# thomasfork/aircraft_trajectory_optimization

Hardware: AMD Instinct MI355X
Metric: SQP iters/sec (batched) + lap-time err vs CasADi, 50×4 collocation (higher is better)
Workload: dtype f64; 1 GPU; racetrack_parametric_esp_drone_colloc_N50_K4_cold_start_batched_sqp; N=50, K=4, nz=13, nu=4, batch_per_gpu=512, global_batch=512, max_iter=47, layout=interleaved, parallelism=instances sharded x1

## Files before the change

### aircraft_trajectory_optimization_amd/csrc/ato_ipm.hip

```cpp
#include <hip/hip_runtime.h>
#include <cmath>
#include <string>
#include "../../include/ato_ipm.h"
#include "../../include/ato.h"

void ato_internal_set_error(const std::string& msg);

namespace {

constexpr int CH = 32;
constexpr int CB = 64;
constexpr int QMAX = 9;

__device__ __forceinline__ double nmax(double a, double b) {
    return (a != a || b != b) ? __builtin_nan("") : (a > b ? a : b);
}
__device__ __forceinline__ double nmin(double a, double b) {
    return (a != a || b != b) ? __builtin_nan("") : (a < b ? a : b);
}
__device__ __forceinline__ bool fin(double v) { return fabs(v) < INFINITY; }

struct Parts {
    int len[4];
    int c0[5];
// ... 580 lines not shown
        filter_reset_step(o, t, n, c, last, k1);
        if (t.ok) {
            ka = k;
            arm = t.arm_case;
            break;
        }
        al = al * 0.5;
    }
    fr_n[p] = n;
    fr_cnt[p] = c;
    fr_last[p] = last ? 1 : 0;
    nf[p] = k1;
    kacc[p] = ka;
    fail_out[p] = fl ? 1 : 0;
    arm_out[p] = arm ? 1 : 0;
}

__global__ __launch_bounds__(256) void k_kkt_diag(Dev d, const double* __restrict__ Sx, const double* __restrict__ Ss,
                                                  const double* __restrict__ dw, const double* __restrict__ dc,
                                                  double* __restrict__ dx, double* __restrict__ dr,
                                                  double* __restrict__ Ds) {
    const long long t = (long long)blockIdx.x * 256 + threadIdx.x;
    const long long nW = (long long)d.n * d.W, iW = (long long)d.mi * d.W, eW = (long long)d.meq * d.W;
    if (t < nW) {
        const int b = (int)(t % d.W);
        dx[t] = Sx[t] + dw[b];
    } else if (t < nW + iW) {
        const long long u = t - nW;
        const int r = (int)(u / d.W), b = (int)(u - (long long)r * d.W);
        const double ds = Ss[u] + dw[b];
// ... 564 lines not shown
    const int k0 = blockIdx.y * RROWS, k1 = min(n0 + m, k0 + RROWS);
    for (int k = k0 + (threadIdx.x >> 6); k < k1; k += 4) {
        const long long o = (long long)k * W + b;
        if (k < n0) {
            x[o] = xb[o];
        } else {
            const long long d = (long long)(k - n0) * W + b;
            const double y = xb[o], rp = x[o], rn = x[o + (long long)m * W];
            x[o] = (rp + y) / dp[d];
            x[o + (long long)m * W] = (rn - y) / dn[d];
            x[o + 2LL * m * W] = y;
        }
    }
}

}

extern "C" {

int ato_ipm_perturb(int32_t op, int32_t W, int32_t m, const double* prm, int64_t* hdeg, int64_t* jdeg,
                    int64_t* diters, int64_t* test, double* dx, double* dc, double* dx_last, double* dc_last,
                    const double* mu, uint8_t* pend, const int32_t* inertia, double* dw_out, double* dc_out,
                    uint8_t* tosolve, const uint8_t* fin, void* stream) {
    if (op < 0 || op > 2 || W < 0 || !prm) return fail(ATO_ERR_ARG, "ato_ipm_perturb: arguments");
    if (W == 0) return 0;
    if (!hdeg || !jdeg || !diters || !test || !dx || !dc || !dx_last || !dc_last || !mu || !pend ||
        (op == 1 && (!inertia || !dw_out || !dc_out || !tosolve)) || (op == 2 && (!tosolve || !fin)))
        return fail(ATO_ERR_ARG, "ato_ipm_perturb: arguments");
    const PertPrm o{prm[0], prm[1], prm[2], prm[3], prm[4], prm[5], prm[6], prm[7], (long long)prm[8]};
    hipLaunchKernelGGL(k_perturb, dim3((W + CB - 1) / CB), dim3(CB), 0, static_cast<hipStream_t>(stream), (int)op, W,
                       m, o, reinterpret_cast<long long*>(hdeg), reinterpret_cast<long long*>(jdeg),
                       reinterpret_cast<long long*>(diters), reinterpret_cast<long long*>(test), dx, dc, dx_last,
                       dc_last, mu, pend, inertia, dw_out, dc_out, tosolve, fin);
// ... 321 lines not shown
```

### aircraft_trajectory_optimization_amd/native.py

```python
import ctypes
import os
from typing import Optional, Tuple

import numpy as np

KMAX = 9
GEOM_WIDTH = 16

ATO_MODEL_DRONE, ATO_MODEL_POINT = 0, 1
ATO_ATT_ESP, ATO_ATT_YPR, ATO_ATT_DCM = 0, 1, 2
ATO_FRAME_GLOBAL, ATO_FRAME_PARAMETRIC = 0, 1
ATO_TRANS_COLLOCATION, ATO_TRANS_RK4 = 0, 1
ATO_GATE_CIRCLE, ATO_GATE_SQUARE = 0, 1
ATO_LAYOUT_INTERLEAVED, ATO_LAYOUT_INSTANCE_MAJOR = 0, 1
ATO_OK, ATO_ERR_ARG, ATO_ERR_UNSUPPORTED, ATO_ERR_HIP, ATO_ERR_STATE = 0, -1, -2, -3, -4
ABI_VERSION = 3
CPC_MAX = 16

_c_double_p = ctypes.POINTER(ctypes.c_double)


class AtoGate(ctypes.Structure):
    _fields_ = [
        ('interval', ctypes.c_int32),
# ... 60 lines not shown

class AtoIpmDims(ctypes.Structure):
    _fields_ = [('n', ctypes.c_int32), ('m', ctypes.c_int32), ('mi', ctypes.c_int32), ('meq', ctypes.c_int32),
                ('iin', ctypes.c_void_p), ('ieq', ctypes.c_void_p), ('W', ctypes.c_int32)]


class AtoIpmBounds(ctypes.Structure):
    _fields_ = [('xL', ctypes.c_void_p), ('xU', ctypes.c_void_p), ('dL', ctypes.c_void_p), ('dU', ctypes.c_void_p)]


IPM_SYMBOLS = ('ato_ipm_work_size', 'ato_ipm_errors', 'ato_ipm_rhs', 'ato_ipm_direction', 'ato_ipm_measures',
               'ato_ipm_multipliers', 'ato_ipm_filter_accept', 'ato_ipm_kkt_diag', 'ato_ipm_perturb',
               'ato_ipm_status', 'ato_ipm_barrier', 'ato_ipm_filter_multi', 'ato_ipm_refine_work',
               'ato_ipm_refine_pass', 'ato_ipm_refine_decide', 'ato_ipm_resto_rows', 'ato_ipm_js_jty',
               'ato_ipm_kmul_residual', 'ato_ipm_resto_eval', 'ato_ipm_resto_hess', 'ato_ipm_resto_kkt_pack',
               'ato_ipm_resto_kkt_diag', 'ato_ipm_resto_kkt_rhs', 'ato_ipm_resto_kkt_expand')

EXPORTED_SYMBOLS = ('ato_create', 'ato_destroy', 'ato_sizes', 'ato_sparsity', 'ato_bounds',
                    'ato_reserve', 'ato_eval', 'ato_eval_f32', 'ato_hess_sparsity', 'ato_hess_eval',
                    'ato_mesh_create', 'ato_mesh_destroy', 'ato_mesh_signed_distance',
                    'ato_timing', 'ato_timing_read', 'ato_timing_stride', 'ato_last_error', 'ato_version',
                    'ato_kkt_create', 'ato_kkt_destroy', 'ato_kkt_reserve', 'ato_kkt_factor', 'ato_kkt_solve',
                    'ato_kkt_residual', 'ato_kkt_residual_list', 'ato_set_instance_spheres',
                    'ato_sphere_rows', 'ato_gradf_mode', 'ato_gradf_sparsity', 'ato_replay_set_lift',
                    'ato_replay', 'ato_remesh') + IPM_SYMBOLS


def library_path() -> str:
    return os.environ.get('ATO_LIB_PATH') or os.path.join(os.path.dirname(os.path.abspath(__file__)), '_lib',
                                                          'libato.so')

# ... 53 lines not shown
        lib.ato_ipm_perturb.argtypes = [ctypes.c_int32] * 3 + [vp] * 16 + [vp]
        lib.ato_ipm_status.argtypes = [ctypes.c_int32] + [vp] * 11 + [vp]
        lib.ato_ipm_barrier.argtypes = [ctypes.c_int32] + [vp] * 10 + [vp]
        lib.ato_ipm_refine_work.argtypes = [ctypes.c_int32, ctypes.c_int32]
        lib.ato_ipm_refine_pass.argtypes = [ctypes.c_int32, ctypes.c_int32] + [vp] * 7 + [vp]
        lib.ato_ipm_refine_decide.argtypes = [ctypes.c_int32] * 4 + [vp] * 12 + [vp]
        lib.ato_ipm_resto_rows.argtypes = [ctypes.c_int32, ctypes.c_int32] + [vp] * 5 + [vp]
        lib.ato_ipm_js_jty.argtypes = [ctypes.c_int32] * 3 + [vp] * 8 + [vp]
        lib.ato_ipm_kmul_residual.argtypes = [ctypes.c_int32] * 5 + [vp] * 15 + [vp]
        lib.ato_ipm_resto_eval.argtypes = [ctypes.c_int32] * 5 + [vp] * 10 + [d] + [vp] * 3 + [vp]
        lib.ato_ipm_resto_hess.argtypes = [ctypes.c_int32] * 2 + [vp] * 7 + [vp]
        lib.ato_ipm_resto_kkt_pack.argtypes = [ctypes.c_int32] * 4 + [vp] * 9 + [vp]
        lib.ato_ipm_resto_kkt_diag.argtypes = [ctypes.c_int32] * 3 + [vp] * 9 + [vp]
        lib.ato_ipm_resto_kkt_rhs.argtypes = [ctypes.c_int32] * 3 + [vp] * 4 + [vp]
        lib.ato_ipm_resto_kkt_expand.argtypes = [ctypes.c_int32] * 3 + [vp] * 5 + [vp]
        for fn in IPM_SYMBOLS[1:]:
            getattr(lib, fn).restype = ctypes.c_int
        for fn in ('ato_create', 'ato_destroy', 'ato_sizes', 'ato_sparsity', 'ato_bounds', 'ato_reserve',
                   'ato_eval', 'ato_eval_f32', 'ato_hess_sparsity', 'ato_hess_eval', 'ato_timing',
                   'ato_timing_read', 'ato_timing_stride', 'ato_mesh_create', 'ato_mesh_destroy', 'ato_mesh_signed_distance',
                   'ato_set_instance_spheres', 'ato_sphere_rows', 'ato_gradf_mode', 'ato_gradf_sparsity',
                   'ato_replay_set_lift', 'ato_replay', 'ato_remesh'):
            getattr(lib, fn).restype = ctypes.c_int
    return lib


_LIB: Optional[ctypes.CDLL] = None


def load(path: Optional[str] = None) -> ctypes.CDLL:
# ... 225 lines not shown
```

### aircraft_trajectory_optimization_amd/solver/batched_ipm.py

```python
import os
import time
from dataclasses import dataclass, field
from typing import Dict, List, Optional

import numpy as np
import torch

from aircraft_trajectory_optimization_amd.solver.ipm import DEG_NO, DEG_UNKNOWN, DEG_YES, INF, IPMOptions, \
    T_C0X0, T_C0XP, T_CPX0, T_CPXP, T_NONE

RUNNING, OPTIMAL, ACCEPTABLE, MAX_ITER, LS_FAILED, KKT_FAILED, STOPPED, INACTIVE, TINY_STEP = range(9)
STATUS_NAMES = {RUNNING: 'running', OPTIMAL: 'optimal', ACCEPTABLE: 'acceptable', MAX_ITER: 'max_iter',
                LS_FAILED: 'restoration_failed', KKT_FAILED: 'kkt_failure', STOPPED: 'stopped',
                INACTIVE: 'inactive', TINY_STEP: 'tiny_step'}
WD_VECS = ('x', 's', 'y', 'zl', 'zu', 'vl', 'vu', 'dx', 'ds', 'dy', 'dzl', 'dzu', 'dvl', 'dvu')
WD_SCAL = ('alpha_max', 'alpha_z', 'theta', 'phi', 'gphi_d')
CSTAT = ('watchdog_started', 'watchdog_reverted', 'soft_resto_steps', 'resto_iterations', 'kkt_failures')
FILTER_MAX = 256


@dataclass
class BatchedIPMResult:
    x: torch.Tensor
    f: torch.Tensor
# ... 588 lines not shown
        al = alpha0.clone()
        for k in range(K):
            inval = act & ~(al > alpha_min)
            failed = failed | inval
            act = act & ~inval
            ok, armk = self._accept(theta, phi, gphi_d, al, tht[k], pht[k], F, nf, theta_min=theta_min, pend=act,
                                    frs=frs, theta_max=theta_max)
            kacc = torch.where(ok, torch.full_like(kacc, k), kacc)
            arm = torch.where(ok, armk, arm)
            act = act & ~ok
            al = al * 0.5
        return kacc, failed, arm

    LS_MULTI_K = int(os.environ.get('ATO_LS_MULTI_K', '8'))
    FUSED_RESTO = os.environ.get('ATO_IPM_FUSED_RESTO', '1') != '0'

    @staticmethod
    def _halvings(K, device):
        return torch.tensor([0.5 ** k for k in range(K)], dtype=torch.float64, device=device)

    def _multi_round(self, idx, P, K, x, s, dx, ds, alpha, alpha_min, mu, theta, phi, gphi_d, F, nf, frs):
        import copy
        cols = idx.repeat(K)
        pw = self._halvings(K + 1, alpha.device)[:K]
        ak = alpha.index_select(0, idx)[None, :] * pw[:, None]
        akf = ak.reshape(-1)
        Xm = x.index_select(1, cols) + akf * dx.index_select(1, cols)
        Sm = s.index_select(1, cols) + akf * ds.index_select(1, cols)
        view = copy.copy(self)
        if self.vk is not None:
            for k in ('sf', 'sg', 'c_rhs', 'xL', 'xU', 'dL', 'dU'):
                t = getattr(self, k)
                if torch.is_tensor(t) and t.dim() >= 1 and t.shape[-1] == self.B:
                    setattr(view, k, t.index_select(t.dim() - 1, cols).contiguous())
        else:
            view._compact(cols, ())
        view.B = K * P
        view.ev = getattr(self.ev, 'trial_subset', getattr(self.ev, 'subset', None))(K * P, cols)
        fm, gm = view._eval_fg(Xm)
        tht, pht = view._measures(Xm, Sm, gm, fm, mu.index_select(0, cols))
        sel = lambda t: t.index_select(0, idx)
        nf_p = sel(nf)
        frs_p = tuple(sel(t) for t in frs)
        kacc, failed, arm = self._filter_multi(sel(theta), sel(phi), sel(gphi_d), sel(alpha), sel(alpha_min),
                                               tht.reshape(K, P).contiguous(), pht.reshape(K, P).contiguous(),
                                               F.index_select(0, idx), nf_p, sel(self.theta_max), sel(self.theta_min),
                                               frs_p)
        nf.index_copy_(0, idx, nf_p)
        for t, tp in zip(frs, frs_p):
            t.index_copy_(0, idx, tp)
        lss = self.stats.setdefault('ls_multi', [0, 0])
        lss[0] += 1
        lss[1] += K * P
        return kacc, failed, arm

    def _filter_test(self, theta, phi, gphi_d, alpha, tht, pht, F, nf, pend, first, frs, theta_min=None):
        tmin = self.theta_min if theta_min is None else theta_min
        if self.vk is not None:
            return self.vk.filter_accept(theta, phi, gphi_d, alpha, tht, pht, F, nf, self.theta_max, tmin, pend,
                                         first, self.o, frs=frs)
        ok, arm = self._accept(theta, phi, gphi_d, alpha, tht, pht, F, nf, theta_min=tmin, pend=pend, frs=frs)
        return ok, arm, pend & ~ok & first & (tht >= theta)

    def _solve(self, rhs, mask, H, Js, dx, dr, idx=None):
        if idx is None:
            idx = _idx(mask)
        x = rhs.clone()
        if len(idx) == 0:
# ... 500 lines not shown
                        self._bd(), x, s, dx, ds, zl, zu, vl, vu, gx, gs, mu, tau)
                else:
                    dzl = torch.where(self.hxl, mu / a - zl - zl / a * dx, 0.0)
                    dzu = torch.where(self.hxu, mu / b - zu + zu / b * dx, 0.0)
                    dvl = torch.where(self.hsl, mu / c - vl - vl / c * ds, 0.0)
                    dvu = torch.where(self.hsu, mu / d - vu + vu / d * ds, 0.0)
                    alpha_max = torch.minimum(
                        torch.minimum(self._ftb(a, dx, self.hxl, tau), self._ftb(b, -dx, self.hxu, tau)),
                        torch.minimum(self._ftb(c, ds, self.hsl, tau), self._ftb(d, -ds, self.hsu, tau)))
                    alpha_z = torch.minimum(
                        torch.minimum(self._ftb(zl, dzl, self.hxl, tau), self._ftb(zu, dzu, self.hxu, tau)),
                        torch.minimum(self._ftb(vl, dvl, self.hsl, tau), self._ftb(vu, dvu, self.hsu, tau)))
                    gphi_d = (gx * dx).sum(0) + (gs * ds).sum(0)
                theta, phi = self._measures(x, s, g, f, mu)
                tiny = torch.zeros_like(act)
                if o.tiny_step_tol > 0:
                    rel_x = (dx.abs() / (1.0 + x.abs())).amax(0) if n else torch.zeros_like(mu)
                    rel_s = (ds.abs() / (1.0 + s.abs())).amax(0) if ds.shape[0] else torch.zeros_like(mu)
                    dymax = dy.abs().amax(0) if m else torch.zeros_like(mu)
                    tiny = act & ~in_wd & ~kwd & (rel_x <= o.tiny_step_tol) & (rel_s <= o.tiny_step_tol) & \
                        (dymax <= o.tiny_step_y_tol) & (theta <= 1e-4)
                    tiny_flag = tiny_flag | tiny
                soft_now = act & in_soft & ~tiny
                soft_count = torch.where(soft_now, soft_count + 1, soft_count)
                soft_over = soft_now & (soft_count > o.max_soft_resto_iters)
                soft_try = soft_now & ~soft_over
                dirs = {'dx': dx, 'ds': ds, 'dy': dy, 'dzl': dzl, 'dzu': dzu, 'dvl': dvl, 'dvu': dvu}
                nosoc = torch.zeros_like(act)
                wdm = torch.zeros_like(act)
                any_kwd = any_wd = False
                if wd_on:
                    start = act & ~tiny & ~in_wd & ~kwd & ~in_soft & (ws_short >= o.watchdog_shortened_iter_trigger)
                    wdm = act & ~kwd & (in_wd | start)
                    any_start, any_kwd, any_wd = torch.stack([start.any(), kwd.any(), wdm.any()]).tolist()
# ... 19 lines not shown
                                                                           ('vu', vu)))
                    for k in dirs:
                        dirs[k] = torch.where(m2, wd[k], dirs[k])
                    alpha_max, alpha_z, theta, phi, gphi_d = (
                        torch.where(msk, wd[k], v) for k, v in (('alpha_max', alpha_max), ('alpha_z', alpha_z),
                                                                ('theta', theta), ('phi', phi), ('gphi_d', gphi_d)))
                    in_wd = in_wd & ~msk
                    nosoc = nosoc | msk
                    fe_, ge_, gfe_, jve_ = self._eval(x)
                    f, g = torch.where(msk, fe_, f), torch.where(m2, ge_, g)
                    gf, jv = torch.where(m2, gfe_, gf), torch.where(m2, jve_, jv)
                    wdst[2] += msk.sum()
                    cst[1] += msk.long()

                def alpha_min_of(theta_, gphi_):
                    neg = gphi_ < 0
                    mgd = torch.clamp(-gphi_, min=1e-300)
                    t1 = o.gamma_phi * theta_ / mgd
                    t2 = o.delta * theta_ ** o.s_theta / mgd ** o.s_phi
                    amin = torch.where(neg & (theta_ <= self.theta_min),
                                       torch.clamp(torch.minimum(t1, t2), max=o.gamma_theta),
                                       torch.where(neg, torch.clamp(t1, max=o.gamma_theta),
                                                   torch.full_like(t1, o.gamma_theta)))
                    return o.alpha_min_frac * amin

                if any_kwd:
                    revert(kwd)
                dx, ds, dy, dzl, dzu, dvl, dvu = (dirs[k] for k in ('dx', 'ds', 'dy', 'dzl', 'dzu', 'dvl', 'dvu'))
                alpha_min = alpha_min_of(theta, gphi_d)
                alpha = torch.where(kwd, alpha_max * 0.5, alpha_max) if any_kwd else alpha_max.clone()
                wd_succ = torch.zeros_like(act)
                wd_cols = wdm.clone()
                pend = act & ~soft_now
                resto = torch.zeros(B, dtype=torch.bool, device=dev)
                first = torch.ones(B, dtype=torch.bool, device=dev)
                xn, sn = x.clone(), s.clone()
                an, dyn = torch.zeros_like(alpha), dy.clone()
                armn = torch.zeros(B, dtype=torch.bool, device=dev)
                fresh = pend.clone()
                fresh_any = True
                accf = torch.zeros(B, dtype=torch.bool, device=dev)
                frs = (fr_n, fr_cnt, fr_last)

                def take(mask, al, xt, st, arm, dyt):
                    nonlocal xn, sn, an, dyn, armn, accf
                    m2 = mask[None, :]
                    xn = torch.where(m2, xt, xn)
                    sn = torch.where(m2, st, sn)
                    an = torch.where(mask, al, an)
                    dyn = torch.where(m2, dyt, dyn)
                    armn = torch.where(mask, arm, armn)
                    accf = torch.where(mask, fresh, accf)

                laps.lap('direction')
                lsfail = torch.zeros_like(act)
                for _ls in range(200):
                    failed = pend & ~(alpha > alpha_min)
                    if o.ls_first_trial:
                        failed = failed & ~fresh
                    any_failed, n_left = torch.stack([failed.any(), (pend & ~failed).sum()]).tolist()
                    if any_failed:
                        lsfail = lsfail | failed
                        pend = pend & ~failed
                    if not n_left:
                        break
                    lss = self.stats.setdefault('ls_trials', [0, 0, 0])
                    lss[0] += 1
                    lss[1] += int(n_left)
                    lss[2] += int(_ls == 0)
                    K = self.LS_MULTI_K
                    if K > 0 and _ls >= 1 and not fresh_any and getattr(self.ev, 'trial_subset_ok',
                                                                          hasattr(self.ev, 'subset')):
                        pidx = torch.nonzero(pend).reshape(-1)
                        kacc, mfail, marm = self._multi_round(pidx, int(n_left), K, x, s, dx, ds, alpha, alpha_min,
                                                              mu, theta, phi, gphi_d, F, nf, frs)
                        acc_p = kacc >= 0
                        a_p = alpha.index_select(0, pidx) * self._halvings(K + 1, dev).index_select(
                            0, torch.where(acc_p, kacc, K).long())
                        acc = torch.zeros_like(pend).index_copy(0, pidx, acc_p)
                        mf = torch.zeros_like(pend).index_copy(0, pidx, mfail)
                        alpha = alpha.index_copy(0, pidx, a_p)
                        take(acc, alpha, x + alpha * dx, s + alpha * ds, torch.zeros_like(pend).index_copy(0, pidx, marm),
                             dy)
                        lsfail = lsfail | mf
                        pend = pend & ~acc & ~mf
                        continue
                    xt = x + alpha * dx
                    st = s + alpha * ds
                    laps.lap('ls_logic')
                    ft, gt = self._eval_fg(xt)
                    laps.lap('ls_eval')
                    tht, pht = self._measures(xt, st, gt, ft, mu)
                    if _ls == 0 and any_wd:
                        th_r, ph_r = torch.where(wdm, wd['theta'], theta), torch.where(wdm, wd['phi'], phi)
                        gd_r, al_r = torch.where(wdm, wd['gphi_d'], gphi_d), torch.where(wdm, wd['alpha_max'], alpha)
                    else:
                        th_r, ph_r, gd_r, al_r = theta, phi, gphi_d, alpha
                    okt, armt, soc = self._filter_test(th_r, ph_r, gd_r, al_r, tht, pht, F, nf,
                                                       pend & ~tiny if _ls == 0 else pend, first, frs)
                    soc = soc & ~nosoc & ~wdm & ~tiny
                    take(okt, alpha, xt, st, armt, dy)
                    pend = pend & ~okt
                    if _ls == 0:
# ... 718 lines not shown
```

### aircraft_trajectory_optimization_amd/solver/ipm_device.py

```python
import ctypes
from typing import Dict, Tuple

import numpy as np
import torch

from aircraft_trajectory_optimization_amd import native


def _p(t):
    return ctypes.c_void_p(t.data_ptr()) if t is not None else None


def resto_rows(dr, dp, dn):
    m, W = dr.shape
    for t in (dr, dp, dn):
        if t.dtype != torch.float64 or t.shape != (m, W) or not t.is_cuda:
            raise ValueError('resto_rows: expected fp64 [m, W] device tensors')
    dr, dp, dn = dr.contiguous(), dp.contiguous(), dn.contiguous()
    drow = torch.empty_like(dr)
    cnt = torch.zeros((W, 2), dtype=torch.int32, device=dr.device)
    lib = native.load()
    rc = lib.ato_ipm_resto_rows(m, W, _p(dr), _p(dp), _p(dn), _p(drow), _p(cnt),
                                ctypes.c_void_p(torch.cuda.current_stream(dr.device).cuda_stream))
    if rc != 0:
# ... 361 lines not shown
        self._own(frs[0], torch.int64, P, 'filter reset count')
        self._own(frs[1], torch.int64, P, 'filter reset trigger count')
        self._own(frs[2], torch.bool, P, 'filter rejection flag')
        key = ('filter', o.s_phi, o.s_theta, o.delta, o.eta_phi, o.gamma_theta, o.gamma_phi, o.obj_max_inc,
               o.compare_tol, o.max_filter_resets, o.filter_reset_trigger)
        prm = self._host_prm(key)
        kacc = torch.empty(P, dtype=torch.int32, device=self.device)
        out = torch.empty((2, P), dtype=torch.bool, device=self.device)
        th, ph, gd, a0, amin, tmax, tmin = cols
        self._check(self.lib.ato_ipm_filter_multi(P, K, F.shape[1], _p(th), _p(ph), _p(gd), _p(a0), _p(amin), _p(tht),
                                                  _p(pht), _p(F), _p(nf), _p(tmax), _p(tmin), prm.ctypes.data,
                                                  _p(frs[0]), _p(frs[1]), _p(frs[2]), _p(kacc), _p(out[0]),
                                                  _p(out[1]), self._stream()), 'ato_ipm_filter_multi')
        return kacc, out[0], out[1]

    def _refine_vec(self, t, N, W, what):
        if t.dtype != torch.float64 or t.device != self.device or t.shape != (N, W) or not t.is_contiguous():
            raise ValueError(f'refinement {what}: expected contiguous fp64 [{N}, {W}] on {self.device}')
        return t

    def refine_begin(self, rhs, x, res, mask, o):
        N, W = rhs.shape
        for t, w in ((rhs, 'rhs'), (x, 'x'), (res, 'residual')):
            self._refine_vec(t, N, W, w)
        self._own(mask, torch.bool, W, 'solved-column mask')
        nch = int(self.lib.ato_ipm_refine_work(N, W))
        f64 = dict(dtype=torch.float64, device=self.device)
        u8 = dict(dtype=torch.bool, device=self.device)
        key = ('refine', o.residual_ratio_max, o.residual_ratio_singular, o.min_refinement_steps,
               o.max_refinement_steps)
# ... 100 lines not shown
```

### include/ato_ipm.h

```cpp
#ifndef ATO_IPM_H
#define ATO_IPM_H

#include <stddef.h>
#include <stdint.h>

#ifdef __cplusplus
extern "C" {
#endif

typedef struct ato_ipm_dims {
    int32_t n;
    int32_t m;
    int32_t mi;
    int32_t meq;
    const int32_t* iin;
    const int32_t* ieq;
    int32_t W;
} ato_ipm_dims;

typedef struct ato_ipm_bounds {
    const double* xL;
    const double* xU;
    const double* dL;
    const double* dU;
// ... 76 lines not shown
                       const double* jv, const double* sg, const double* x_ref, const double* dr2,
                       const double* zeta, double rho, double* gr, double* gfr, double* jr, void* stream);
int ato_ipm_resto_hess(int32_t nnz, int32_t W, const int32_t* src, const int32_t* dcol, const double* H0,
                       const double* sigma, const double* zeta, const double* dr2, double* h, void* stream);
int ato_ipm_resto_kkt_pack(int32_t nh, int32_t nj, int32_t n0, int32_t W, const int32_t* h_map,
                           const int32_t* pos_orig, const int32_t* h_diag, const uint8_t* diag_new, const double* H,
                           const double* J, double* Hb, double* Jb, double* hd, void* stream);
int ato_ipm_resto_kkt_diag(int32_t n0, int32_t m, int32_t W, const double* dx, const double* dr, const double* hd,
                           const uint8_t* mask, double* dxb, double* drow, double* dp, double* dn, int32_t* cnt,
                           void* stream);
int ato_ipm_resto_kkt_rhs(int32_t n0, int32_t m, int32_t W, const double* x, const double* dp, const double* dn,
                          double* xb, void* stream);
int ato_ipm_resto_kkt_expand(int32_t n0, int32_t m, int32_t W, const double* xb, const double* dp, const double* dn,
                             const uint8_t* mask, double* x, void* stream);

#ifdef __cplusplus
}
#endif
#endif
```

Measured before the change: 6917 SQP iterations/s (instance-iterations of the batched interior-point solve, all GPUs).

## Move line-search trial, acceptance, and step bookkeeping into fused device kernels

Adds HIP kernels for the filter line search: building trial points (optionally gathered through a column map), filter acceptance over an index list that updates alpha in place, copying accepted trials, compacting still-pending instances, a tiny-step max reduction, and alpha_min. The aim is to replace many small torch ops and host-side compaction on each line-search iteration with a few launches that stay on the device. This adds more custom code and depends on the Python driver calling the new wrappers; the driver changes are only partly visible.

```diff
diff --git a/aircraft_trajectory_optimization_amd/csrc/ato_ipm.hip b/aircraft_trajectory_optimization_amd/csrc/ato_ipm.hip
--- a/aircraft_trajectory_optimization_amd/csrc/ato_ipm.hip
+++ b/aircraft_trajectory_optimization_amd/csrc/ato_ipm.hip
@@ -618,6 +618,59 @@
     kacc[p] = ka;
     fail_out[p] = fl ? 1 : 0;
     arm_out[p] = arm ? 1 : 0;
+}
+
+__global__ __launch_bounds__(CB) void k_filter_multi_idx(int P, int K, int W, int fmax, const int32_t* __restrict__ idx,
+                                                         const double* __restrict__ theta,
+                                                         const double* __restrict__ phi,
+                                                         const double* __restrict__ gphi_d,
+                                                         double* __restrict__ alpha,
+                                                         const double* __restrict__ alpha_min,
+                                                         const double* __restrict__ tht,
+                                                         const double* __restrict__ pht, const double* __restrict__ F,
+                                                         int64_t* __restrict__ nf,
+                                                         const double* __restrict__ theta_max,
+                                                         const double* __restrict__ theta_min, FilterPrm o,
+                                                         int64_t* __restrict__ fr_n, int64_t* __restrict__ fr_cnt,
+                                                         uint8_t* __restrict__ fr_last, uint8_t* __restrict__ acc_out,
+                                                         uint8_t* __restrict__ fail_out,
+                                                         uint8_t* __restrict__ arm_out) {
+    const int p = blockIdx.x * CB + threadIdx.x;
+    if (p >= P) return;
+    const int c = idx[p];
+    if (c < 0 || c >= W) return;
+    const double th = theta[c], ph = phi[c], gd = gphi_d[c], amin = alpha_min[c];
+    const double tmax = theta_max[c], tmin = theta_min[c];
+    const double* Fb = F + (long long)c * fmax * 2;
+    long long n = fr_n[c], cn = fr_cnt[c], k1 = nf[c];
+    bool last = fr_last[c] != 0;
+    int ka = -1;
+    bool fl = false, arm = false;
+    const double al0 = alpha[c];
+    double al = al0;
+    for (int k = 0; k < K; ++k) {
+        if (!(al > amin)) {
+            fl = true;
+            break;
+        }
+        const TrialTest t = filter_trial(o, th, ph, gd, al, tht[(long long)k * P + p], pht[(long long)k * P + p], Fb,
+                                         k1, fmax, tmax, tmin);
+        filter_reset_step(o, t, n, cn, last, k1);
+        if (t.ok) {
+            ka = k;
+            arm = t.arm_case;
+            break;
+        }
+        al = al * 0.5;
+    }
+    fr_n[c] = n;
+    fr_cnt[c] = cn;
+    fr_last[c] = last ? 1 : 0;
+    nf[c] = k1;
+    alpha[c] = al0 * ldexp(1.0, -(ka >= 0 ? ka : K));
+    acc_out[c] = ka >= 0 ? 1 : 0;
+    fail_out[c] = fl ? 1 : 0;
+    arm_out[c] = arm ? 1 : 0;
 }
 
 __global__ __launch_bounds__(256) void k_kkt_diag(Dev d, const double* __restrict__ Sx, const double* __restrict__ Ss,
@@ -1212,9 +1265,280 @@
     }
 }
 
+
+__global__ __launch_bounds__(256) void k_ls_trial(int n, int mi, int Wi, int Wo, const int32_t* __restrict__ cols,
+                                                  const double* __restrict__ fac, const double* __restrict__ x,
+                                                  const double* __restrict__ s, const double* __restrict__ dx,
+                                                  const double* __restrict__ ds, double* __restrict__ xt,
+                                                  double* __restrict__ st) {
+#pragma clang fp contract(off)
+    const int b = blockIdx.x * 64 + (threadIdx.x & 63);
+    if (b >= Wo) return;
+    const int c = cols ? cols[b] : b;
+    if (c < 0 || c >= Wi) return;
+    const double a = fac[b];
+    const int k0 = blockIdx.y * RROWS, k1 = min(n + mi, k0 + RROWS);
+    for (int k = k0 + (threadIdx.x >> 6); k < k1; k += 4) {
+        if (k < n) {
+            const long long i = (long long)k * Wi + c;
+            const double p = a * dx[i];
+            xt[(long long)k * Wo + b] = x[i] + p;
+        } else {
+            const long long i = (long long)(k - n) * Wi + c;
+            const double p = a * ds[i];
+            st[(long long)(k - n) * Wo + b] = s[i] + p;
+        }
+    }
+}
+
+__global__ __launch_bounds__(256) void k_ls_take(int n, int mi, int m, int W, const uint8_t* __restrict__ mask,
+                                                 const double* __restrict__ al, const double* __restrict__ xt,
+                                                 const double* __restrict__ st, const uint8_t* __restrict__ arm,
+                                                 const double* __restrict__ dyt, const uint8_t* __restrict__ fresh,
+                                                 double* __restrict__ xn, double* __restrict__ sn,
+                                                 double* __restrict__ an, double* __restrict__ dyn,
+                                                 uint8_t* __restrict__ armn, uint8_t* __restrict__ accf) {
+    const int b = blockIdx.x * 64 + (threadIdx.x & 63);
+    if (b >= W || !mask[b]) return;
+    if (blockIdx.y == 0 && threadIdx.x < 64) {
+        an[b] = al[b];
+        armn[b] = arm ? (arm[b] ? 1 : 0) : 1;
+        accf[b] = fresh[b] ? 1 : 0;
+    }
+    const int k0 = blockIdx.y * RROWS, k1 = min(n + mi + m, k0 + RROWS);
+    for (int k = k0 + (threadIdx.x >> 6); k < k1; k += 4) {
+        if (k < n) {
+            const long long i = (long long)k * W + b;
+            xn[i] = xt[i];
+        } else if (k < n + mi) {
+            const long long i = (long long)(k - n) * W + b;
+            sn[i] = st[i];
+        } else {
+            const long long i = (long long)(k - n - mi) * W + b;
+            dyn[i] = dyt[i];
+        }
+    }
+}
+
+__global__ __launch_bounds__(RD_THREADS) void k_ls_advance(int W, const double* __restrict__ alpha,
+                                                           const double* __restrict__ alpha_min,
+                                                           const uint8_t* __restrict__ fresh,
+                                                           uint8_t* __restrict__ pend, uint8_t* __restrict__ lsfail,
+                                                           int32_t* __restrict__ info) {
+    __shared__ int wcount[RD_THREADS / 64];
+    __shared__ int total, anyf;
+    const int tid = threadIdx.x, lane = tid & 63, wv = tid >> 6;
+    if (tid == 0) {
+        total = 0;
+        anyf = 0;
+    }
+    __syncthreads();
+    for (int base = 0; base < W; base += RD_THREADS) {
+        const int col = base + tid;
+        bool flag = false, fl = false;
+        if (col < W) {
+            const bool p = pend[col] != 0;
+            fl = p && !(alpha[col] > alpha_min[col]) && !(fresh && fresh[col] != 0);
+            flag = p && !fl;
+            if (fl) {
+                lsfail[col] = 1;
+                pend[col] = 0;
+            }
+        }
+        const unsigned long long bal = __ballot(flag);
+        const unsigned long long bfl = __ballot(fl);
+        if (lane == 0) {
+            wcount[wv] = __popcll(bal);
+            if (bfl) anyf = 1;
+        }
+        __syncthreads();
+        int off = total;
+        for (int w = 0; w < wv; ++w) off += wcount[w];
+        if (flag) info[2 + off + __popcll(bal & ((1ull << lane) - 1ull))] = col;
+        __syncthreads();
+        if (tid == 0) {
+            int t = total;
+            for (int w = 0; w < RD_THREADS / 64; ++w) t += wcount[w];
+            total = t;
+        }
+        __syncthreads();
+    }
+    if (tid == 0) {
+        info[0] = anyf;
+        info[1] = total;
+    }
+}
+
+__global__ __launch_bounds__(256) void k_tiny_pass(int n, int mi, int m, int W, int rows, const double* __restrict__ x,
+                                                   const double* __restrict__ s, const double* __restrict__ dx,
+                                                   const double* __restrict__ ds, const double* __restrict__ dy,
+                                                   double* __restrict__ part) {
+#pragma clang fp contract(off)
+    __shared__ double sq[3][4][64];
+    const int lane = threadIdx.x & 63, wv = threadIdx.x >> 6;
+    const int col = blockIdx.x * 64 + lane;
+    const int r0 = blockIdx.y * rows, r1 = min(n + mi + m, r0 + rows);
+    double q0 = 0.0, q1 = 0.0, q2 = 0.0;
+    if (col < W) {
+        for (int r = r0 + wv; r < r1; r += 4) {
+            if (r < n) {
+                const long long i = (long long)r * W + col;
+                const double den = 1.0 + fabs(x[i]);
+                q0 = nmax(q0, fabs(dx[i]) / den);
+            } else if (r < n + mi) {
+                const long long i = (long long)(r - n) * W + col;
+                const double den = 1.0 + fabs(s[i]);
+                q1 = nmax(q1, fabs(ds[i]) / den);
+            } else {
+                q2 = nmax(q2, fabs(dy[(long long)(r - n - mi) * W + col]));
+            }
+        }
+    }
+    sq[0][wv][lane] = q0;
+    sq[1][wv][lane] = q1;
+    sq[2][wv][lane] = q2;
+    __syncthreads();
+    if (wv == 0 && col < W) {
+        const int nch = gridDim.y;
+#pragma unroll
+        for (int q = 0; q < 3; ++q)
+            part[((long long)q * nch + blockIdx.y) * W + col] =
+                nmax(nmax(sq[q][0][lane], sq[q][1][lane]), nmax(sq[q][2][lane], sq[q][3][lane]));
+    }
+}
+
+__global__ __launch_bounds__(CB) void k_tiny_fold(int W, int nch, const double* __restrict__ part,
+                                                  double* __restrict__ out) {
+    const int b = blockIdx.x * CB + threadIdx.x;
+    if (b >= W) return;
+#pragma unroll
+    for (int q = 0; q < 3; ++q) {
+        double v = 0.0;
+        for (int c = 0; c < nch; ++c) v = nmax(v, part[((long long)q * nch + c) * W + b]);
+        out[(long long)q * W + b] = v;
+    }
+}
+
+struct AlphaMinPrm {
+    double gamma_phi, delta, s_theta, s_phi, gamma_theta, alpha_min_frac;
+};
+
+__device__ __forceinline__ double cmin_(double a, double b) { return a != a ? a : (a > b ? b : a); }
+
+__global__ __launch_bounds__(CB) void k_alpha_min(int W, AlphaMinPrm o, const double* __restrict__ theta,
+                                                  const double* __restrict__ gphi_d,
+                                                  const double* __restrict__ theta_min, double* __restrict__ out) {
+#pragma clang fp contract(off)
+    const int b = blockIdx.x * CB + threadIdx.x;
+    if (b >= W) return;
+    const double th = theta[b], gd = gphi_d[b];
+    const bool neg = gd < 0.0;
+    const double mgd = cmax(-gd, 1e-300);
+    const double t1 = (o.gamma_phi * th) / mgd;
+    const double t2 = (o.delta * tpow(th, o.s_theta)) / tpow(mgd, o.s_phi);
+    double amin;
+    if (neg && th <= theta_min[b]) amin = cmin_(nmin(t1, t2), o.gamma_theta);
+    else if (neg) amin = cmin_(t1, o.gamma_theta);
+    else amin = o.gamma_theta;
+    out[b] = o.alpha_min_frac * amin;
+}
+
 }
 
 extern "C" {
+
+int ato_ipm_ls_trial(int32_t n, int32_t mi, int32_t Wi, int32_t Wo, const int32_t* cols, const double* fac,
+                     const double* x, const double* s, const double* dx, const double* ds, double* xt, double* st,
+                     void* stream) {
+    if (n < 0 || mi < 0 || Wi < 0 || Wo < 0 || (!cols && Wi != Wo))
+        return fail(ATO_ERR_ARG, "ato_ipm_ls_trial: arguments");
+    if (Wo == 0 || n + mi == 0) return 0;
+    if (Wi == 0 || !fac || (n && (!x || !dx || !xt)) || (mi && (!s || !ds || !st)))
+        return fail(ATO_ERR_ARG, "ato_ipm_ls_trial: arguments");
+    if ((n + mi + RROWS - 1) / RROWS > GRID_Y_MAX) return fail(ATO_ERR_ARG, "ato_ipm_ls_trial: too many rows");
+    hipLaunchKernelGGL(k_ls_trial, dim3((Wo + 63) / 64, (n + mi + RROWS - 1) / RROWS), dim3(256), 0,
+                       static_cast<hipStream_t>(stream), n, mi, Wi, Wo, cols, fac, x, s, dx, ds, xt, st);
+    return check_launch("ato_ipm_ls_trial");
+}
+
+int ato_ipm_ls_take(int32_t n, int32_t mi, int32_t m, int32_t W, const uint8_t* mask, const double* al,
+                    const double* xt, const double* st, const uint8_t* arm, const double* dyt, const uint8_t* fresh,
+                    double* xn, double* sn, double* an, double* dyn, uint8_t* armn, uint8_t* accf, void* stream) {
+    if (n < 0 || mi < 0 || m < 0 || W < 0) return fail(ATO_ERR_ARG, "ato_ipm_ls_take: arguments");
+    if (W == 0) return 0;
+    if (!mask || !al || !fresh || !an || !armn || !accf || (n && (!xt || !xn)) || (mi && (!st || !sn)) ||
+        (m && (!dyt || !dyn)))
+        return fail(ATO_ERR_ARG, "ato_ipm_ls_take: arguments");
+    const int rows = n + mi + m;
+    const int ny = rows ? (rows + RROWS - 1) / RROWS : 1;
+    if (ny > GRID_Y_MAX) return fail(ATO_ERR_ARG, "ato_ipm_ls_take: too many rows");
+    hipLaunchKernelGGL(k_ls_take, dim3((W + 63) / 64, ny), dim3(256), 0, static_cast<hipStream_t>(stream), n, mi, m,
+                       W, mask, al, xt, st, arm, dyt, fresh, xn, sn, an, dyn, armn, accf);
+    return check_launch("ato_ipm_ls_take");
+}
+
+int ato_ipm_ls_advance(int32_t W, const double* alpha, const double* alpha_min, const uint8_t* fresh, uint8_t* pend,
+                       uint8_t* lsfail, int32_t* info, void* stream) {
+    if (W < 0 || !info || (W && (!alpha || !alpha_min || !pend || !lsfail)))
+        return fail(ATO_ERR_ARG, "ato_ipm_ls_advance: arguments");
+    hipLaunchKernelGGL(k_ls_advance, dim3(1), dim3(RD_THREADS), 0, static_cast<hipStream_t>(stream), W, alpha,
+                       alpha_min, fresh, pend, lsfail, info);
+    return check_launch("ato_ipm_ls_advance");
+}
+
+int ato_ipm_filter_multi_idx(int32_t P, int32_t K, int32_t W, int32_t fmax, const int32_t* idx, const double* theta,
+                             const double* phi, const double* gphi_d, double* alpha, const double* alpha_min,
+                             const double* tht, const double* pht, const double* F, int64_t* nf,
+                             const double* theta_max, const double* theta_min, const double* prm, int64_t* fr_n,
+                             int64_t* fr_cnt, uint8_t* fr_last, uint8_t* acc, uint8_t* failed, uint8_t* arm,
+                             void* stream) {
+    if (P < 0 || K < 1 || K > 1000 || W < 0 || P > W || fmax < 0 || !prm)
+        return fail(ATO_ERR_ARG, "ato_ipm_filter_multi_idx: arguments");
+    if (P == 0) return 0;
+    if (!idx || !theta || !phi || !gphi_d || !alpha || !alpha_min || !tht || !pht || (fmax && !F) || !nf ||
+        !theta_max || !theta_min || !fr_n || !fr_cnt || !fr_last || !acc || !failed || !arm)
+        return fail(ATO_ERR_ARG, "ato_ipm_filter_multi_idx: arguments");
+    const FilterPrm o{prm[0], prm[1], prm[2], prm[3], prm[4], prm[5], prm[6], prm[7], (long long)prm[8],
+                      (long long)prm[9]};
+    hipLaunchKernelGGL(k_filter_multi_idx, dim3((P + CB - 1) / CB), dim3(CB), 0, static_cast<hipStream_t>(stream), P,
+                       K, W, fmax, idx, theta, phi, gphi_d, alpha, alpha_min, tht, pht, F, nf, theta_max, theta_min,
+                       o, fr_n, fr_cnt, fr_last, acc, failed, arm);
+    return check_launch("ato_ipm_filter_multi_idx");
+}
+
+int ato_ipm_tiny_work(int32_t rows) {
+    if (rows <= 0) return 1;
+    const int nch = (rows + 63) / 64;
+    return nch < 64 ? nch : 64;
+}
+
+int ato_ipm_tiny_step(int32_t n, int32_t mi, int32_t m, int32_t W, const double* x, const double* s, const double* dx,
+                      const double* ds, const double* dy, double* part, double* out, void* stream) {
+    if (n < 0 || mi < 0 || m < 0 || W < 0 || (long long)n + mi + m > 0x7fffffffLL)
+        return fail(ATO_ERR_ARG, "ato_ipm_tiny_step: arguments");
+    if (W == 0) return 0;
+    if (!part || !out || (n && (!x || !dx)) || (mi && (!s || !ds)) || (m && !dy))
+        return fail(ATO_ERR_ARG, "ato_ipm_tiny_step: arguments");
+    const int total = n + mi + m;
+    const int nch = ato_ipm_tiny_work(total);
+    const int rows = total ? (total + nch - 1) / nch : 0;
+    auto st = static_cast<hipStream_t>(stream);
+    hipLaunchKernelGGL(k_tiny_pass, dim3((W + 63) / 64, nch), dim3(256), 0, st, n, mi, m, W, rows, x, s, dx, ds, dy,
+                       part);
+    hipLaunchKernelGGL(k_tiny_fold, dim3((W + CB - 1) / CB), dim3(CB), 0, st, W, nch, part, out);
+    return check_launch("ato_ipm_tiny_step");
+}
+
+int ato_ipm_alpha_min(int32_t W, const double* prm, const double* theta, const double* gphi_d,
+                      const double* theta_min, double* out, void* stream) {
+    if (W < 0 || !prm) return fail(ATO_ERR_ARG, "ato_ipm_alpha_min: arguments");
+    if (W == 0) return 0;
+    if (!theta || !gphi_d || !theta_min || !out) return fail(ATO_ERR_ARG, "ato_ipm_alpha_min: arguments");
+    const AlphaMinPrm o{prm[0], prm[1], prm[2], prm[3], prm[4], prm[5]};
+    hipLaunchKernelGGL(k_alpha_min, dim3((W + CB - 1) / CB), dim3(CB), 0, static_cast<hipStream_t>(stream), W, o,
+                       theta, gphi_d, theta_min, out);
+    return check_launch("ato_ipm_alpha_min");
+}
 
 int ato_ipm_perturb(int32_t op, int32_t W, int32_t m, const double* prm, int64_t* hdeg, int64_t* jdeg,
                     int64_t* diters, int64_t* test, double* dx, double* dc, double* dx_last, double* dc_last,
diff --git a/aircraft_trajectory_optimization_amd/native.py b/aircraft_trajectory_optimization_amd/native.py
--- a/aircraft_trajectory_optimization_amd/native.py
+++ b/aircraft_trajectory_optimization_amd/native.py
@@ -98,7 +98,9 @@
                'ato_ipm_status', 'ato_ipm_barrier', 'ato_ipm_filter_multi', 'ato_ipm_refine_work',
                'ato_ipm_refine_pass', 'ato_ipm_refine_decide', 'ato_ipm_resto_rows', 'ato_ipm_js_jty',
                'ato_ipm_kmul_residual', 'ato_ipm_resto_eval', 'ato_ipm_resto_hess', 'ato_ipm_resto_kkt_pack',
-               'ato_ipm_resto_kkt_diag', 'ato_ipm_resto_kkt_rhs', 'ato_ipm_resto_kkt_expand')
+               'ato_ipm_resto_kkt_diag', 'ato_ipm_resto_kkt_rhs', 'ato_ipm_resto_kkt_expand', 'ato_ipm_ls_trial',
+               'ato_ipm_ls_take', 'ato_ipm_ls_advance', 'ato_ipm_filter_multi_idx', 'ato_ipm_tiny_work', 'ato_ipm_tiny_step',
+               'ato_ipm_alpha_min')
 
 EXPORTED_SYMBOLS = ('ato_create', 'ato_destroy', 'ato_sizes', 'ato_sparsity', 'ato_bounds',
                     'ato_reserve', 'ato_eval', 'ato_eval_f32', 'ato_hess_sparsity', 'ato_hess_eval',
@@ -182,6 +184,13 @@
         lib.ato_ipm_resto_kkt_diag.argtypes = [ctypes.c_int32] * 3 + [vp] * 9 + [vp]
         lib.ato_ipm_resto_kkt_rhs.argtypes = [ctypes.c_int32] * 3 + [vp] * 4 + [vp]
         lib.ato_ipm_resto_kkt_expand.argtypes = [ctypes.c_int32] * 3 + [vp] * 5 + [vp]
+        lib.ato_ipm_ls_trial.argtypes = [ctypes.c_int32] * 4 + [vp] * 8 + [vp]
+        lib.ato_ipm_ls_take.argtypes = [ctypes.c_int32] * 4 + [vp] * 13 + [vp]
+        lib.ato_ipm_ls_advance.argtypes = [ctypes.c_int32] + [vp] * 6 + [vp]
+        lib.ato_ipm_filter_multi_idx.argtypes = [ctypes.c_int32] * 4 + [vp] * 19 + [vp]
+        lib.ato_ipm_tiny_work.argtypes = [ctypes.c_int32]
+        lib.ato_ipm_tiny_step.argtypes = [ctypes.c_int32] * 4 + [vp] * 7 + [vp]
+        lib.ato_ipm_alpha_min.argtypes = [ctypes.c_int32] + [vp] * 5 + [vp]
         for fn in IPM_SYMBOLS[1:]:
             getattr(lib, fn).restype = ctypes.c_int
         for fn in ('ato_create', 'ato_destroy', 'ato_sizes', 'ato_sparsity', 'ato_bounds', 'ato_reserve',
diff --git a/aircraft_trajectory_optimization_amd/solver/batched_ipm.py b/aircraft_trajectory_optimization_amd/solver/batched_ipm.py
--- a/aircraft_trajectory_optimization_amd/solver/batched_ipm.py
+++ b/aircraft_trajectory_optimization_amd/solver/batched_ipm.py
@@ -626,19 +626,26 @@
 
     LS_MULTI_K = int(os.environ.get('ATO_LS_MULTI_K', '8'))
     FUSED_RESTO = os.environ.get('ATO_IPM_FUSED_RESTO', '1') != '0'
+    FUSED_LS = os.environ.get('ATO_IPM_FUSED_LS', '1') != '0'
+
+    def _fused_ls(self, t):
+        return self.FUSED_LS and self.vk is not None and t.is_cuda
 
     @staticmethod
     def _halvings(K, device):
         return torch.tensor([0.5 ** k for k in range(K)], dtype=torch.float64, device=device)
 
-    def _multi_round(self, idx, P, K, x, s, dx, ds, alpha, alpha_min, mu, theta, phi, gphi_d, F, nf, frs):
+    def _multi_round(self, idx, P, K, x, s, dx, ds, alpha, alpha_min, mu, theta, phi, gphi_d, F, nf, frs, idx32=None):
         import copy
         cols = idx.repeat(K)
         pw = self._halvings(K + 1, alpha.device)[:K]
         ak = alpha.index_select(0, idx)[None, :] * pw[:, None]
         akf = ak.reshape(-1)
-        Xm = x.index_select(1, cols) + akf * dx.index_select(1, cols)
-        Sm = s.index_select(1, cols) + akf * ds.index_select(1, cols)
+        if self._fused_ls(x):
+            Xm, Sm = self.vk.ls_trial(x, s, dx, ds, akf, cols.to(torch.int32))
+        else:
+            Xm = x.index_select(1, cols) + akf * dx.index_select(1, cols)
+            Sm = s.index_select(1, cols) + akf * ds.index_select(1, cols)
         view = copy.copy(self)
         if self.vk is not None:
             for k in ('sf', 'sg', 'c_rhs', 'xL', 'xU', 'dL', 'dU'):
@@ -651,6 +658,13 @@
         view.ev = getattr(self.ev, 'trial_subset', getattr(self.ev, 'subset', None))(K * P, cols)
         fm, gm = view._eval_fg(Xm)
         tht, pht = view._measures(Xm, Sm, gm, fm, mu.index_select(0, cols))
+        lss = self.stats.setdefault('ls_multi', [0, 0])
+        lss[0] += 1
+        lss[1] += K * P
+        if idx32 is not None:
+            return self.vk.filter_multi_idx(idx32, theta, phi, gphi_d, alpha, alpha_min,
+                                            tht.reshape(K, P).contiguous(), pht.reshape(K, P).contiguous(), F, nf,
+                                            self.theta_max, self.theta_min, self.o, frs)
         sel = lambda t: t.index_select(0, idx)
         nf_p = sel(nf)
         frs_p = tuple(sel(t) for t in frs)
@@ -661,9 +675,6 @@
         nf.index_copy_(0, idx, nf_p)
         for t, tp in zip(frs, frs_p):
             t.index_copy_(0, idx, tp)
-        lss = self.stats.setdefault('ls_multi', [0, 0])
-        lss[0] += 1
-        lss[1] += K * P
         return kacc, failed, arm
 
     def _filter_test(self, theta, phi, gphi_d, alpha, tht, pht, F, nf, pend, first, frs, theta_min=None):
@@ -1194,10 +1205,14 @@
                     gphi_d = (gx * dx).sum(0) + (gs * ds).sum(0)
                 theta, phi = self._measures(x, s, g, f, mu)
                 tiny = torch.zeros_like(act)
+                fused_ls = self._fused_ls(x)
                 if o.tiny_step_tol > 0:
-                    rel_x = (dx.abs() / (1.0 + x.abs())).amax(0) if n else torch.zeros_like(mu)
-                    rel_s = (ds.abs() / (1.0 + s.abs())).amax(0) if ds.shape[0] else torch.zeros_like(mu)
-                    dymax = dy.abs().amax(0) if m else torch.zeros_like(mu)
+                    if fused_ls:
+                        rel_x, rel_s, dymax = self.vk.tiny_step(x, s, dx, ds, dy)
+                    else:
+                        rel_x = (dx.abs() / (1.0 + x.abs())).amax(0) if n else torch.zeros_like(mu)
+                        rel_s = (ds.abs() / (1.0 + s.abs())).amax(0) if ds.shape[0] else torch.zeros_like(mu)
+                        dymax = dy.abs().amax(0) if m else torch.zeros_like(mu)
                     tiny = act & ~in_wd & ~kwd & (rel_x <= o.tiny_step_tol) & (rel_s <= o.tiny_step_tol) & \
                         (dymax <= o.tiny_step_y_tol) & (theta <= 1e-4)
                     tiny_flag = tiny_flag | tiny
@@ -1247,6 +1262,8 @@
                     cst[1] += msk.long()
 
                 def alpha_min_of(theta_, gphi_):
+                    if fused_ls:
+                        return self.vk.alpha_min(theta_, gphi_, self.theta_min, o)
                     neg = gphi_ < 0
                     mgd = torch.clamp(-gphi_, min=1e-300)
                     t1 = o.gamma_phi * theta_ / mgd
@@ -1277,6 +1294,9 @@
 
                 def take(mask, al, xt, st, arm, dyt):
                     nonlocal xn, sn, an, dyn, armn, accf
+                    if fused_ls:
+                        self.vk.ls_take(mask, al, xt, st, arm, dyt, fresh, xn, sn, an, dyn, armn, accf)
+                        return
                     m2 = mask[None, :]
                     xn = torch.where(m2, xt, xn)
                     sn = torch.where(m2, st, sn)
@@ -1288,13 +1308,18 @@
                 laps.lap('direction')
                 lsfail = torch.zeros_like(act)
                 for _ls in range(200):
-                    failed = pend & ~(alpha > alpha_min)
-                    if o.ls_first_trial:
-                        failed = failed & ~fresh
-                    any_failed, n_left = torch.stack([failed.any(), (pend & ~failed).sum()]).tolist()
-                    if any_failed:
-                        lsfail = lsfail | failed
-                        pend = pend & ~failed
+                    if fused_ls:
+                        ls_info = self.vk.ls_advance(alpha, alpha_min, fresh if o.ls_first_trial else None, pend,
+                                                     lsfail)
+                        any_failed, n_left = ls_info[:2].tolist()
+                    else:
+                        failed = pend & ~(alpha > alpha_min)
+                        if o.ls_first_trial:
+                            failed = failed & ~fresh
+                        any_failed, n_left = torch.stack([failed.any(), (pend & ~failed).sum()]).tolist()
+                        if any_failed:
+                            lsfail = lsfail | failed
+                            pend = pend & ~failed
                     if not n_left:
                         break
                     lss = self.stats.setdefault('ls_trials', [0, 0, 0])
@@ -1304,7 +1329,16 @@
                     K = self.LS_MULTI_K
                     if K > 0 and _ls >= 1 and not fresh_any and getattr(self.ev, 'trial_subset_ok',
                                                                           hasattr(self.ev, 'subset')):
-                        pidx = torch.nonzero(pend).reshape(-1)
+                        pidx = ls_info[2:2 + n_left].long() if fused_ls else torch.nonzero(pend).reshape(-1)
+                        if fused_ls:
+                            acc, mf, marm = self._multi_round(pidx, int(n_left), K, x, s, dx, ds, alpha, alpha_min,
+                                                              mu, theta, phi, gphi_d, F, nf, frs,
+                                                              idx32=ls_info[2:2 + n_left])
+                            xa, sa = self.vk.ls_trial(x, s, dx, ds, alpha)
+                            take(acc, alpha, xa, sa, marm, dy)
+                            lsfail = lsfail | mf
+                            pend = pend & ~acc & ~mf
+                            continue
                         kacc, mfail, marm = self._multi_round(pidx, int(n_left), K, x, s, dx, ds, alpha, alpha_min,
                                                               mu, theta, phi, gphi_d, F, nf, frs)
                         acc_p = kacc >= 0
@@ -1318,8 +1352,11 @@
                         lsfail = lsfail | mf
                         pend = pend & ~acc & ~mf
                         continue
-                    xt = x + alpha * dx
-                    st = s + alpha * ds
+                    if fused_ls:
+                        xt, st = self.vk.ls_trial(x, s, dx, ds, alpha)
+                    else:
+                        xt = x + alpha * dx
+                        st = s + alpha * ds
                     laps.lap('ls_logic')
                     ft, gt = self._eval_fg(xt)
                     laps.lap('ls_eval')
diff --git a/aircraft_trajectory_optimization_amd/solver/ipm_device.py b/aircraft_trajectory_optimization_amd/solver/ipm_device.py
--- a/aircraft_trajectory_optimization_amd/solver/ipm_device.py
+++ b/aircraft_trajectory_optimization_amd/solver/ipm_device.py
@@ -399,6 +399,101 @@
                                                   _p(out[1]), self._stream()), 'ato_ipm_filter_multi')
         return kacc, out[0], out[1]
 
+    def _mask(self, t, W, what):
+        if t.dtype != torch.bool or t.device != self.device or t.shape != (W,):
+            raise ValueError(f'{what}: expected bool [{W}] on {self.device}')
+        return t.contiguous()
+
+    def ls_trial(self, x, s, dx, ds, fac, cols=None):
+        n, mi = self.n, self.mi
+        Wi = x.shape[1]
+        x, s, dx, ds = self._v(x, n, Wi), self._v(s, mi, Wi), self._v(dx, n, Wi), self._v(ds, mi, Wi)
+        if cols is None:
+            Wo = Wi
+        else:
+            Wo = cols.shape[0]
+            if cols.dtype != torch.int32 or cols.dim() != 1 or cols.device != self.device or not cols.is_contiguous():
+                raise ValueError('ls_trial: the column map must be a contiguous int32 vector on the device')
+        fac = self._c(fac, Wo)
+        xt = torch.empty((n, Wo), dtype=torch.float64, device=self.device)
+        st = torch.empty((mi, Wo), dtype=torch.float64, device=self.device)
+        self._check(self.lib.ato_ipm_ls_trial(n, mi, Wi, Wo, _p(cols), _p(fac), _p(x), _p(s), _p(dx), _p(ds), _p(xt),
+                                              _p(st), self._stream()), 'ato_ipm_ls_trial')
+        return xt, st
+
+    def ls_take(self, mask, al, xt, st, arm, dyt, fresh, xn, sn, an, dyn, armn, accf):
+        n, mi, m = self.n, self.mi, self.m
+        W = mask.shape[0]
+        for t, rows, what in ((xn, n, 'xn'), (sn, mi, 'sn'), (dyn, m, 'dyn')):
+            self._refine_vec(t, rows, W, f'ls_take {what}')
+        self._own(an, torch.float64, W, 'ls_take an')
+        self._own(armn, torch.bool, W, 'ls_take armn')
+        self._own(accf, torch.bool, W, 'ls_take accf')
+        ops = [self._mask(mask, W, 'ls_take mask'), self._c(al, W), self._v(xt, n, W), self._v(st, mi, W),
+               None if arm is None else self._mask(arm, W, 'ls_take arm'), self._v(dyt, m, W),
+               self._mask(fresh, W, 'ls_take fresh')]
+        self._check(self.lib.ato_ipm_ls_take(n, mi, m, W, *[_p(t) for t in ops], _p(xn), _p(sn), _p(an), _p(dyn),
+                                             _p(armn), _p(accf), self._stream()), 'ato_ipm_ls_take')
+
+    def ls_advance(self, alpha, alpha_min, fresh, pend, lsfail):
+        W = pend.shape[0]
+        self._own(pend, torch.bool, W, 'ls_advance pend')
+        self._own(lsfail, torch.bool, W, 'ls_advance lsfail')
+        info = torch.empty(W + 2, dtype=torch.int32, device=self.device)
+        self._check(self.lib.ato_ipm_ls_advance(W, _p(self._c(alpha, W)), _p(self._c(alpha_min, W)),
+                                                None if fresh is None else _p(self._mask(fresh, W, 'ls_advance fresh')),
+                                                _p(pend), _p(lsfail), _p(info), self._stream()), 'ato_ipm_ls_advance')
+        return info
+
+    def filter_multi_idx(self, idx, theta, phi, gphi_d, alpha, alpha_min, tht, pht, F, nf, theta_max, theta_min, o,
+                         frs):
+        W = theta.shape[0]
+        K, P = tht.shape
+        if idx.dtype != torch.int32 or idx.shape != (P,) or idx.device != self.device or not idx.is_contiguous():
+            raise ValueError('filter_multi_idx: the column list must be a contiguous int32 [P] device tensor')
+        cols = [self._c(t, W) for t in (theta, phi, gphi_d, alpha_min, theta_max, theta_min)]
+        self._own(alpha, torch.float64, W, 'filter_multi_idx alpha')
+        for t in (tht, pht):
+            if t.dtype != torch.float64 or t.shape != (K, P) or not t.is_contiguous() or t.device != self.device:
+                raise ValueError('filter_multi_idx: trial measures must be contiguous fp64 [K, P]')
+        if F.dtype != torch.float64 or F.shape[0] != W or F.dim() != 3 or F.shape[2] != 2 or not F.is_contiguous():
+            raise ValueError('filter: expected contiguous fp64 [W, fmax, 2]')
+        self._own(nf, torch.int64, W, 'filter length')
+        self._own(frs[0], torch.int64, W, 'filter reset count')
+        self._own(frs[1], torch.int64, W, 'filter reset trigger count')
+        self._own(frs[2], torch.bool, W, 'filter rejection flag')
+        prm = self._host_prm(('filter', o.s_phi, o.s_theta, o.delta, o.eta_phi, o.gamma_theta, o.gamma_phi,
+                              o.obj_max_inc, o.compare_tol, o.max_filter_resets, o.filter_reset_trigger))
+        out = torch.zeros((3, W), dtype=torch.bool, device=self.device)
+        th, ph, gd, amin, tmax, tmin = cols
+        self._check(self.lib.ato_ipm_filter_multi_idx(P, K, W, F.shape[1], _p(idx), _p(th), _p(ph), _p(gd), _p(alpha),
+                                                      _p(amin), _p(tht), _p(pht), _p(F), _p(nf), _p(tmax), _p(tmin),
+                                                      prm.ctypes.data, _p(frs[0]), _p(frs[1]), _p(frs[2]), _p(out[0]),
+                                                      _p(out[1]), _p(out[2]), self._stream()),
+                    'ato_ipm_filter_multi_idx')
+        return out[0], out[1], out[2]
+
+    def tiny_step(self, x, s, dx, ds, dy):
+        n, mi, m = self.n, self.mi, self.m
+        W = x.shape[1]
+        ops = [self._v(x, n, W), self._v(s, mi, W), self._v(dx, n, W), self._v(ds, mi, W), self._v(dy, m, W)]
+        nch = int(self.lib.ato_ipm_tiny_work(n + mi + m))
+        part = torch.empty((3, nch, W), dtype=torch.float64, device=self.device)
+        out = torch.empty((3, W), dtype=torch.float64, device=self.device)
+        self._check(self.lib.ato_ipm_tiny_step(n, mi, m, W, *[_p(t) for t in ops], _p(part), _p(out),
+                                               self._stream()), 'ato_ipm_tiny_step')
+        return out[0], out[1], out[2]
+
+    def alpha_min(self, theta, gphi_d, theta_min, o):
+        W = theta.shape[0]
+        prm = self._host_prm(('alpha_min', o.gamma_phi, o.delta, o.s_theta, o.s_phi, o.gamma_theta,
+                              o.alpha_min_frac))
+        out = torch.empty(W, dtype=torch.float64, device=self.device)
+        self._check(self.lib.ato_ipm_alpha_min(W, prm.ctypes.data, _p(self._c(theta, W)), _p(self._c(gphi_d, W)),
+                                               _p(self._c(theta_min, W)), _p(out), self._stream()),
+                    'ato_ipm_alpha_min')
+        return out
+
     def _refine_vec(self, t, N, W, what):
         if t.dtype != torch.float64 or t.device != self.device or t.shape != (N, W) or not t.is_contiguous():
             raise ValueError(f'refinement {what}: expected contiguous fp64 [{N}, {W}] on {self.device}')
diff --git a/include/ato_ipm.h b/include/ato_ipm.h
--- a/include/ato_ipm.h
+++ b/include/ato_ipm.h
@@ -114,6 +114,26 @@
 int ato_ipm_resto_kkt_expand(int32_t n0, int32_t m, int32_t W, const double* xb, const double* dp, const double* dn,
                              const uint8_t* mask, double* x, void* stream);
 
+int ato_ipm_ls_trial(int32_t n, int32_t mi, int32_t Wi, int32_t Wo, const int32_t* cols, const double* fac,
+                     const double* x, const double* s, const double* dx, const double* ds, double* xt, double* st,
+                     void* stream);
+int ato_ipm_ls_take(int32_t n, int32_t mi, int32_t m, int32_t W, const uint8_t* mask, const double* al,
+                    const double* xt, const double* st, const uint8_t* arm, const double* dyt, const uint8_t* fresh,
+                    double* xn, double* sn, double* an, double* dyn, uint8_t* armn, uint8_t* accf, void* stream);
+int ato_ipm_ls_advance(int32_t W, const double* alpha, const double* alpha_min, const uint8_t* fresh, uint8_t* pend,
+                       uint8_t* lsfail, int32_t* info, void* stream);
+int ato_ipm_filter_multi_idx(int32_t P, int32_t K, int32_t W, int32_t fmax, const int32_t* idx, const double* theta,
+                             const double* phi, const double* gphi_d, double* alpha, const double* alpha_min,
+                             const double* tht, const double* pht, const double* F, int64_t* nf,
+                             const double* theta_max, const double* theta_min, const double* prm, int64_t* fr_n,
+                             int64_t* fr_cnt, uint8_t* fr_last, uint8_t* acc, uint8_t* failed, uint8_t* arm,
+                             void* stream);
+int ato_ipm_tiny_work(int32_t rows);
+int ato_ipm_tiny_step(int32_t n, int32_t mi, int32_t m, int32_t W, const double* x, const double* s, const double* dx,
+                      const double* ds, const double* dy, double* part, double* out, void* stream);
+int ato_ipm_alpha_min(int32_t W, const double* prm, const double* theta, const double* gphi_d,
+                      const double* theta_min, double* out, void* stream);
+
 #ifdef __cplusplus
 }
 #endif
```

After: 6475 SQP iterations/s (instance-iterations of the batched interior-point solve, all GPUs). 0.936x the previous value.
